# jagannatharjun/AntiZ

Hardware: AMD Instinct MI355X
Metric: input MB/s precompressed (1 GB synthetic, 100k streams) at 1/2/4/8 MI355X (higher is better)
Workload: dtype u8

## Files before the change

antiz_amd/__init__.py:

```python
import ctypes as C
import os

HERE = os.path.dirname(os.path.abspath(__file__))
LIB_PATH = os.environ.get("ATZ_LIB") or os.path.join(HERE, "_build", "libatz_accel.so")
CLI_PATH = os.path.join(HERE, "_build", "uncomp")

u64 = C.c_uint64
u8p = C.POINTER(C.c_uint8)


class Opts(C.Structure):
    _fields_ = [("recomp_tresh", u64), ("sizediff_tresh", u64), ("shortcut_len", u64), ("mismatch_tol", u64),
                ("chunksize", u64), ("brute_window", C.c_int32), ("device", C.c_int32)]


class Cand(C.Structure):
    _fields_ = [("offset", u64), ("comp_len", u64), ("infl_len", u64), ("type", C.c_int32), ("flags", C.c_uint32)]


class Result(C.Structure):
    _fields_ = [("clevel", C.c_uint8), ("window", C.c_uint8), ("memlevel", C.c_uint8), ("recomp", C.c_uint8),
                ("n_trials", C.c_uint32), ("ident", u64), ("first_diff", C.c_int64), ("n_diff", u64),
                ("diff_index", u64)]

# ... 12 lines not shown
                                   "trial_cyc_heap", "trial_cyc_fallback", "trial_symbols",
                                   "n_trials_speculative", "n_reinflated", "n_inflate_retries", "n_trials_replayed", "n_replay_checked",
                                   "n_trials_duplicate", "n_fast_restarts", "dev_bytes_peak", "dev_bytes_held",
                                   "n_trials_skipped")]

    def as_dict(self):
        return {k: getattr(self, k) for k, _ in self._fields_}


EXPORTS = ["atz_open", "atz_close", "atz_strerror", "atz_free", "atz_default_opts", "atz_scan", "atz_sweep",
           "atz_precompress", "atz_precompress_device", "atz_reconstruct", "atz_deflate", "atz_deflate_batch",
           "atz_inflate_batch", "atz_deflate_bound", "atz_shard_scan", "atz_shard_sweep", "atz_shard_piece",
           "atz_shard_assemble", "atz_reconstruct_device", "atz_deflate_batch_ex", "atz_set_strategies",
           "atz_set_containers", "atz_container_anchors", "atz_set_stitch", "atz_stitch_anchors",
           "atz_stitch_pieces", "atz_set_probe", "atz_probe_positions", "atz_set_deflaters",
           "atz_set_segments", "atz_flush_markers", "atz_inflate_segments"]

STRATEGIES = {"filtered": 1, "huffman": 2, "rle": 3}


def _mask(names, table, noun):
    if isinstance(names, str):
        names = [w for w in names.split(",") if w]
    mask = 0
    for w in names:
        if w not in table:
            raise ValueError("unknown %s %r (known: %s)" % (noun, w, ", ".join(sorted(table))))
        mask |= 1 << table[w]
    return mask


# ... 110 lines not shown
        L.atz_container_anchors.argtypes = [C.c_void_p, C.c_char_p, u64, C.c_uint32, C.POINTER(C.POINTER(u64)),
                                            C.POINTER(u64)]
        L.atz_set_stitch.argtypes = [C.c_void_p, C.c_uint32]
        L.atz_stitch_anchors.argtypes = L.atz_container_anchors.argtypes
        L.atz_stitch_pieces.argtypes = [C.c_void_p, u64, C.POINTER(C.POINTER(u64)), C.POINTER(C.POINTER(u64)),
                                        C.POINTER(u64)]
        L.atz_set_probe.argtypes = [C.c_void_p, C.c_uint32]
        L.atz_probe_positions.argtypes = [C.c_void_p, C.c_char_p, u64, C.POINTER(C.POINTER(u64)), C.POINTER(u64)]
        L.atz_set_deflaters.argtypes = [C.c_void_p, C.c_uint32]
        L.atz_set_segments.argtypes = [C.c_void_p, C.c_uint32]
        L.atz_flush_markers.argtypes = L.atz_probe_positions.argtypes
        L.atz_inflate_segments.argtypes = [C.c_void_p, C.c_char_p, u64, C.POINTER(u64), C.POINTER(u64), u64,
                                           C.POINTER(C.c_uint32), C.POINTER(u64), C.POINTER(u64), C.POINTER(C.c_uint8)]
        L.atz_deflate_bound.restype = u64
        L.atz_deflate_bound.argtypes = [u64, C.c_int, C.c_int]
        L.atz_shard_scan.argtypes = [C.c_void_p, C.c_void_p, C.c_char_p, u64, C.c_int, C.c_int, C.POINTER(u8p),
                                     C.POINTER(u64)]
        L.atz_shard_sweep.argtypes = [C.c_void_p, C.c_void_p, C.c_char_p, u64, C.POINTER(C.c_char_p),
                                      C.POINTER(u64), C.c_int, C.POINTER(u64), C.POINTER(u8p), C.POINTER(u64),
                                      C.POINTER(u64), C.POINTER(Stats)]
        L.atz_shard_piece.argtypes = [C.c_void_p, C.c_void_p]
        L.atz_reconstruct_device.argtypes = [C.c_void_p, C.c_void_p, C.c_char_p, u64, C.POINTER(C.c_void_p),
                                             C.POINTER(u64)]
        L.atz_shard_assemble.argtypes = [C.c_void_p, C.c_void_p, u64, C.c_char_p, u64, u64, u64, C.c_void_p, u64,
                                         C.POINTER(u64)]
        _lib = L
    return _lib


def _check(rc):
    if rc != 0:
        raise AtzError("atz error %d: %s" % (rc, lib().atz_strerror(rc).decode()), rc)


class Context:

    def __init__(self, recomp_tresh=128, sizediff_tresh=128, shortcut_len=512, mismatch_tol=2,
                 chunksize=524288, brute_window=False, device=-1, strategies=None, containers=None, stitch=None,
                 probe=None, deflaters=None, segments=None):
        L = lib()
        self.o = Opts(recomp_tresh, sizediff_tresh, shortcut_len, mismatch_tol, chunksize, int(brute_window), device)
        if strategies is None:
            strategies = os.environ.get("ATZ_STRATEGIES", "")
        mask = strategy_mask(strategies)
        if containers is None:
            containers = os.environ.get("ATZ_CONTAINERS", "")
        cmask = container_mask(containers)
# ... 235 lines not shown
```

antiz_amd/csrc/atz_accel.cpp:

```cpp
#include "k_inflate.hip"
#include "k_deflate.hip"

#include <algorithm>
#include <array>
#include <chrono>
#include <cstdio>
#include <cstdlib>
#include <cstring>
#include <deque>
#include <string>
#include <memory>
#include <new>
#include <stdexcept>
#include <atomic>
#include <thread>
#include <condition_variable>
#include <mutex>
#include <functional>
#include <unordered_map>
#include <vector>
#include <dlfcn.h>
#include <signal.h>
#include <sys/time.h>
#include <ucontext.h>
// ... 2105 lines not shown
      std::stable_sort(S.perm[k].begin(), S.perm[k].end(), [&](uint32_t a, uint32_t b) {
        const bool ma = mw_trial(c, k, in[k][a].memlevel), mb = mw_trial(c, k, in[k][b].memlevel);
        return ma != mb ? ma : key[a] > key[b];
      });
    }
    if (strat)
      std::stable_sort(S.perm[k].begin(), S.perm[k].end(), [&](uint32_t a, uint32_t b) {
        return trial_variant(c, k, in[k][a]) < trial_variant(c, k, in[k][b]);
      });
    S.tr[k].resize(n);
    for (size_t q = 0; q < n; q++) S.tr[k][q] = in[k][S.perm[k][q]];
    S.res[k].clear();
  }
  S.base = 0;
}
static int trials_launch(atz_ctx* x, Pipe* c, const uint8_t* d_cmp, const SweepOpts& so, int k, const Trial* h,
                         size_t cnt, size_t base) {
  struct Kern { int kind; uint32_t strat; bool mw; void (*fn)(SweepArgs); const char* name; };
  static const Kern kerns[] = {
      {0, 0, false, k_trial_stored, "k_trial_stored"},
      {0, 2, false, k_trial_huff, "k_trial_huff"},
      {0, 3, false, k_trial_rle, "k_trial_rle"},
      {1, 0, true, k_trial_fast_mw<BITMAP_BITS>, "k_trial_fast"},
      {1, 0, false, k_trial_fast<BITMAP_BITS>, "k_trial_fast"},
      {2, 0, true, k_trial_slow_mw, "k_trial_slow"},
      {2, 0, false, k_trial_slow, "k_trial_slow"},
      {2, 1, true, k_trial_slow_filt_mw, "k_trial_slow_filt"},
      {2, 1, false, k_trial_slow_filt, "k_trial_slow_filt"},
      {1, 4, false, k_trial_fast_gnu, "k_trial_fast_gnu"},
      {2, 4, false, k_trial_slow_gnu, "k_trial_slow_gnu"},
      {0, 8, false, k_trial_stored_flush, "k_trial_stored_flush"},
      {1, 8, true, k_trial_fast_flush_mw, "k_trial_fast_flush"},
      {1, 8, false, k_trial_fast_flush, "k_trial_fast_flush"},
      {2, 8, true, k_trial_slow_flush_mw, "k_trial_slow_flush"},
      {2, 8, false, k_trial_slow_flush, "k_trial_slow_flush"},
  };
  for (size_t i = 0; i < cnt; i++)
    if (h[i].host & (TH_WAITS | TH_DUP)) return ATZ_E_INTERNAL;
  for (size_t i = 0; i < cnt;) {
    const bool mw = mw_trial(c, k, h[i].memlevel);
    size_t j = i + 1;
    while (j < cnt && mw_trial(c, k, h[j].memlevel) == mw) j++;
    HIPCHK(pipe_copy(c, c->d_trials.as<Trial>() + base + i, h + i, (j - i) * sizeof(Trial), hipMemcpyHostToDevice));
    i = j;
  }
  auto launch1 = [&](const Trial* hh, size_t n1, size_t b1, uint32_t variant) -> int {
    (void)hh;
    const bool mw = variant & 1u;
    const Kern* kn = nullptr;
    for (const Kern& e : kerns)
      if (e.kind == k && e.strat == variant >> 1 && e.mw == mw) kn = &e;
    if (!kn) return ATZ_E_INTERNAL;
    SweepArgs A;
    A.file = d_cmp; A.infl = INFL_BASE; A.chains = CHAIN_BASE;
    A.R = c->d_R.as<uint2>();
    A.streams = x->d_streams.as<StreamDev>(); A.trials = c->d_trials.as<Trial>() + b1;
    A.res = c->d_tres.as<TrialRes>() + b1; A.out = c->d_out.as<uint8_t>(); A.syms = c->d_syms.as<uint32_t>();
    A.adler = x->d_adler.as<uint32_t>(); A.o = so; A.ntrials = (uint32_t)n1;
    A.stopj = c->stopj_cur;
    dim3 g((uint32_t)n1), b(mw ? MW_THREADS : 64);
    kbeg(c, variant & 8u ? 5 : 0);
    hipLaunchKernelGGL(kn->fn, g, b, 0, c->st, A);
    kend(c);
    KCHECK(kn->name);
    return 0;
// ... 2186 lines not shown
    uint64_t al = 0;
    auto tc = std::chrono::steady_clock::now();
    if (int r = precompress_dev(c, d_file, h_file, len, &al, nullptr)) return r;
    if (timing_on())
      std::fprintf(stderr, "atz: precompress call %.2f ms (inside: %.2f ms)\n", ms_since(tc), c->stats.total_ms);
    *d_atz = c->d_atz.as<uint8_t>();
    *atz_len = al;
    c->stats.dev_bytes_peak = g_dev.peak.load(); c->stats.dev_bytes_held = g_dev.cur.load();
    if (stats) *stats = c->stats;
    return ATZ_OK;
  });
}

uint64_t atz_deflate_bound(uint64_t n, int window, int memlevel) { return bound(n, window, memlevel); }

int atz_deflate(atz_ctx_t* c, const uint8_t* in, uint64_t in_len, int clevel, int window, int memlevel,
                uint8_t* out, uint64_t out_cap, uint64_t* out_len) {
  return guarded([&]() -> int {
    (void)hipGetLastError();
    if (!c || (!in && in_len) || !out_len || clevel < 0 || clevel > 9 || window < 8 || window > 15 ||
        memlevel < 1 || memlevel > 9)
      return ATZ_E_ARG;
    DeflSpec p;
    p.level = clevel; p.window = window == 8 ? 9 : window; p.memlevel = memlevel;
    std::vector<std::vector<uint8_t>> outs;
    if (int r = deflate_many(c, {{in, in_len}}, {p}, outs)) return r;
    *out_len = outs[0].size();
    if (outs[0].size() > out_cap) return ATZ_E_ARG;
    if (out && !outs[0].empty()) std::memcpy(out, outs[0].data(), outs[0].size());
    return ATZ_OK;
// ... 289 lines not shown
```

antiz_amd/csrc/k_deflate.hip:

```cpp
#include <hip/hip_runtime.h>
#include "atz_device.h"

#define LDS __attribute__((address_space(3)))
#define CONSTANT __attribute__((address_space(4)))
#define GLOBAL __attribute__((address_space(1)))

#ifndef ATZ_VISITED_CHECK
#define ATZ_VISITED_CHECK 1
#endif
#ifndef ATZ_VISITED_MAX
#define ATZ_VISITED_MAX 8
#endif
#ifndef ATZ_NOSLIDE_PATH
#define ATZ_NOSLIDE_PATH 1
#endif
#ifndef ATZ_STEP_SPLIT
#define ATZ_STEP_SPLIT 0
#endif
#ifndef ATZ_STEP_CLOCKS
#define ATZ_STEP_CLOCKS 0
#endif
#if ATZ_STEP_CLOCKS
#define STEP_CLOCK() clock64()
#else
// ... 696 lines not shown
      }
    }
    uint2 o;
    o.x = (bf > 2 ? (bf << 23) | (df << 8) : 0u) | s0;
    if (jb.fast) o.y = ((p - reach) << 16) | (budget_out << 12) | (slot << 1) | valid;
    else o.y = (bq > 2 ? (bq << 23) | (dq << 8) : 0u) | valid;
    r[p] = o;
  }
}

static constexpr int NLC = 286, NDC = 30, NBLC = 19, HEAPN = 2 * NLC + 1;
static constexpr uint32_t LOOKMIN = 262;
static constexpr uint32_t BITMAP_BITS = 32768;
static constexpr uint32_t HOLE_SLOTS = HOLE_SLOTS_M;

struct TreeWork {
  uint32_t heap[HEAPN + 1];
  uint16_t bl_count[16];
  uint32_t blc32[16];
};

struct TreeScratch {
  uint16_t anc[2][HEAPN];
  uint8_t dep[2][HEAPN];
  uint16_t freq[NLC];
};

struct BitOut {
  GLOBAL uint8_t* out;
  uint64_t cap;
  uint64_t pos;
  uint64_t bb;
  uint32_t bc;
  uint32_t raw;
  const GLOBAL uint8_t* orig;
  uint64_t clen;
  uint64_t shortcut;
  uint64_t eq_all;
  uint64_t eq_sc;
  int overflow;
  uint64_t cyc_tree, cyc_emit, blocks;
  uint64_t cyc_heap, cyc_scan, cyc_send;
};

static constexpr uint32_t STAGE_WORDS = 196;
struct BlockFreq {
  uint32_t lfreq2[(NLC + 1) / 2];
  uint32_t dfreq2[NDC / 2];
};
struct TreeCodes {
  uint16_t lcode[NLC]; uint8_t llen[NLC + 2];
  uint16_t dcode[NDC]; uint8_t dlen[NDC + 2];
  uint16_t bcode[NBLC]; uint8_t blen[NBLC + 2];
  uint32_t bfreq[NBLC];
  TreeWork w;
};
struct TrialShared {
  BitOut b;
  BlockFreq f;
  TreeCodes k;
  uint64_t stop_at;
  uint32_t stop_j, pad_;
};

template <uint32_t INS>
struct TrialSharedFast {
  static constexpr uint32_t INS_BITS = INS;
  TrialShared t;
  uint64_t ring[512];
  uint32_t ins[INS / 32];
  uint32_t holes[HOLE_SLOTS];
// ... 189 lines not shown
struct TreeRes {
  int max_code;
  uint64_t d_opt, d_static;
};

__device__ __noinline__ TreeRes build_tree(LDS TreeWork& w, LDS TreeScratch& sc, LDS uint8_t* lenv, int elems, int max_length, const CONSTANT uint8_t* xbits,
                                           int xbase, const CONSTANT uint8_t* stlen, LDS uint64_t& cyc_heap, int lane) {
  elems = (int)uni((uint32_t)elems);
  max_length = (int)uni((uint32_t)max_length);
  xbase = (int)uni((uint32_t)xbase);
  xbits = uni_ptr(xbits);
  stlen = uni_ptr(stlen);
  uint64_t opt_len = 0, static_len = 0;
  const uint64_t lt = lane ? (~0ull >> (64 - lane)) : 0ull;
  LDS uint32_t* const heap = w.heap;
  int heap_len = 0, max_code = -1;
  for (int g = 0; g < elems; g += 64) {
    const int n = g + lane;
    const uint32_t f = n < elems ? sc.freq[n] : 0u;
    const uint64_t m = __ballot(f != 0);
    if (f) heap[heap_len + 1 + __popcll(m & lt)] = tkey(f, 0, (uint32_t)n);
    else if (n < elems) lenv[n] = 0;
    if (m) max_code = g + 63 - __clzll((long long)m);
    heap_len += __popcll(m);
  }
  while (heap_len < 2) {
    const int node = max_code < 2 ? ++max_code : 0;
    ++heap_len;
    if (lane == 0) { heap[heap_len] = tkey(1, 0, (uint32_t)node); sc.freq[node] = 1; }
    opt_len--;
// ... 19 lines not shown
        go = vk > (hj >> 10);
        if (go) { wr(k, hj); k = j; j = k << 1; go = j <= len; }
      }
      wr(k, v);
    };
    for (int n = heap_len / 2; n >= 1; n--) down(heap_len, n);
    do {
      const uint32_t kn = rd(1);
      wr(1, rd(heap_len));
      wr(heap_len, 0xffffffffu);
      heap_len--;
      down(heap_len, 1);
      const uint32_t km = rd(1);
      const uint32_t dn = (kn >> 10) & 31u, dm = (km >> 10) & 31u;
      if (lane == 0) {
        heap[--heap_max] = kn & 1023u;
        heap[--heap_max] = km & 1023u;
        sc.anc[1][kn & 1023u] = (uint16_t)node;
        sc.anc[1][km & 1023u] = (uint16_t)node;
      } else {
        heap_max -= 2;
      }
      wr(1, tkey((kn >> 15) + (km >> 15), (dn >= dm ? dn : dm) + 1u, node));
      node++;
      down(heap_len, 1);
    } while (heap_len >= 2);
    root = rd(1) & 1023u;
  } else {
  for (int n = heap_len / 2; n >= 1; n--) pq_down(heap, heap_len, n, lane);
  do {
    const uint32_t kn = uni(heap[1]);
    heap[1] = uni(heap[heap_len]);
    heap_len--;
    pq_down(heap, heap_len, 1, lane);
    const uint32_t km = uni(heap[1]);
    const uint32_t dn = (kn >> 10) & 31u, dm = (km >> 10) & 31u;
    if (lane == 0) {
      heap[--heap_max] = kn & 1023u;
      heap[--heap_max] = km & 1023u;
      sc.anc[1][kn & 1023u] = (uint16_t)node;
      sc.anc[1][km & 1023u] = (uint16_t)node;
    } else {
      heap_max -= 2;
    }
    heap[1] = tkey((kn >> 15) + (km >> 15), (dn >= dm ? dn : dm) + 1u, node);
    node++;
    pq_down(heap, heap_len, 1, lane);
  } while (heap_len >= 2);
  root = uni(heap[1]) & 1023u;
  }
  if (lane == 0) cyc_heap += STEP_CLOCK() - ch0;
  --heap_max;
  if (lane == 0) heap[heap_max] = root;
  const int nn = (int)node;
  for (int i = lane; i < nn; i += 64) {
    const bool in_tree = i >= elems || (i <= max_code && sc.freq[i] != 0);
    const bool r = (uint32_t)i == root || !in_tree;
    sc.anc[0][i] = r ? (uint16_t)root : sc.anc[1][i];
    sc.dep[0][i] = r ? 0 : 1;
  }
  int cur = 0;
  for (int round = 0; round < 5; round++) {
    for (int i = lane; i < nn; i += 64) {
      const uint32_t a = sc.anc[cur][i];
      sc.dep[cur ^ 1][i] = (uint8_t)(sc.dep[cur][i] + sc.dep[cur][a]);
      sc.anc[cur ^ 1][i] = sc.anc[cur][a];
    }
    cur ^= 1;
  }
  if (lane < 16) w.blc32[lane] = 0;
  int overflow = 0;
  for (int g = 0; g < nn; g += 64) {
    const int i = g + lane;
    bool in_tree = false;
    uint32_t bits = 0;
    if (i < nn) {
      in_tree = i >= elems || (i <= max_code && sc.freq[i] != 0);
      bits = sc.dep[cur][i];
    }
    const bool capped = in_tree && (uint32_t)i != root && bits > (uint32_t)max_length;
    overflow += __popcll(__ballot(capped));
    if (bits > (uint32_t)max_length) bits = (uint32_t)max_length;
    const bool leaf = in_tree && i <= max_code;
    if (leaf) {
      lenv[i] = (uint8_t)bits;
      __hip_atomic_fetch_add(&w.blc32[bits], 1u, __ATOMIC_RELAXED, __HIP_MEMORY_SCOPE_WORKGROUP);
    }
  }
  uint32_t blc = lane >= 1 && lane < 16 ? w.blc32[lane] : 0u;
  if (overflow) {
    auto bl = [&](int b) -> uint32_t { return (uint32_t)__builtin_amdgcn_readlane((int)blc, b); };
    auto blset = [&](int b, uint32_t v) { blc = lane == b ? v : blc; };
    do {
      int bits = max_length - 1;
      while (bl(bits) == 0) bits--;
      blset(bits, bl(bits) - 1);
      blset(bits + 1, bl(bits + 1) + 2);
      blset(max_length, bl(max_length) - 1);
      overflow -= 2;
    } while (overflow > 0);
    int h = HEAPN;
    for (int bits = max_length; bits != 0; bits--) {
      uint32_t cnt = bl(bits);
      while (cnt != 0) {
        const uint32_t m = uni(heap[--h]);
        if ((int)m > max_code) continue;
        if (lane == 0) lenv[m] = (uint8_t)bits;
        cnt--;
      }
    }
  }
  if (lane < 16) w.bl_count[lane] = (uint16_t)blc;
  uint64_t o = 0, st = 0;
  for (int n = lane; n < elems && n <= max_code; n += 64) {
    const uint32_t f = sc.freq[n];
    if (f) {
      const uint32_t l = lenv[n];
      const uint32_t xb = (xbits && n >= xbase) ? xbits[n - xbase] : 0u;
      o += (uint64_t)f * (l + xb);
      if (stlen) st += (uint64_t)f * (stlen[n] + xb);
    }
  }
  opt_len += wsum64(o);
  if (stlen) static_len += wsum64(st);
  return TreeRes{max_code, opt_len, static_len};
}

__device__ __noinline__ void gen_codes(const LDS TreeWork& w, int max_code, LDS uint16_t* codes, LDS uint8_t* lens,
                                       int lane) {
  max_code = (int)uni((uint32_t)max_code);
  const bool lb = lane >= 1 && lane <= 15;
  const uint32_t bc = lb ? (uint32_t)w.bl_count[lane] : 0u;
  const uint32_t wv = bc << ((15 - lane) & 15);
  uint32_t nc = lb ? (wave_incl_scan(wv) - wv) >> (15 - lane) : 0u;
  const uint64_t lt = lane ? (~0ull >> (64 - lane)) : 0ull;
  const uint64_t present = __ballot(bc != 0);
  for (int g = 0; g <= max_code; g += 64) {
    const int n = g + lane;
    const uint32_t l = n <= max_code ? lens[n] : 0u;
    uint32_t mine = 0;
    for (uint64_t pm = present; pm; pm &= pm - 1) {
      const int b = __ffsll((unsigned long long)pm) - 1;
      const uint64_t m = __ballot(l == (uint32_t)b);
      if (!m) continue;
      const uint32_t base = (uint32_t)__builtin_amdgcn_readlane((int)nc, b);
      if (l == (uint32_t)b) mine = base + (uint32_t)__popcll(m & lt);
      if (lane == b) nc += (uint32_t)__popcll(m);
// ... 59 lines not shown
      if (xd) { v |= (uint64_t)(dist - dcode_base(dcd)) << nb; nb += xd; }
    }
  } else if (end) {
    v = lc[256]; nb = ll[256];
  }
}
__device__ __forceinline__ void stage_or(LDS uint32_t* stage, uint32_t off, uint64_t v, uint32_t nb) {
  if (!nb) return;
  const uint32_t wi = off >> 5, sh = off & 31;
  const uint64_t lo = v << sh;
  const uint32_t hi = sh ? (uint32_t)(v >> (64 - sh)) : 0;
  __atomic_fetch_or(&stage[wi], (uint32_t)lo, __ATOMIC_RELAXED);
  if ((uint32_t)(lo >> 32)) __atomic_fetch_or(&stage[wi + 1], (uint32_t)(lo >> 32), __ATOMIC_RELAXED);
  if (hi) __atomic_fetch_or(&stage[wi + 2], hi, __ATOMIC_RELAXED);
}
__device__ uint32_t rle_tree(LDS TreeCodes& s, LDS uint32_t* stage, const LDS uint8_t* ln, int max_code, bool send,
                             uint32_t off, int lane) {
  const int N = max_code + 1;
  const int G = N / 64 + 1;
  uint64_t M[5];
#pragma unroll
  for (int g = 0; g < 5; g++) {
    M[g] = 0;
    if (g < G) {
      const int n = 64 * g + lane;
      bool st = false;
      if (n == 0 || n == N) st = true;
      else if (n < N) st = ln[n] != ln[n - 1];
      M[g] = __ballot(st);
    }
  }
// ... 16 lines not shown
          const uint64_t m = h == g ? (M[h] & ~le) : M[h];
          if (m) en = 64 * h + __ffsll((unsigned long long)m) - 1;
        }
      const uint32_t v = ln[n];
      const int k = n - st, R = en - st;
      int cnt = 0, minc = 3;
      bool first = false;
      if (v != 0) {
        if (k == 0) { cnt = R < 7 ? R : 7; minc = 4; first = true; }
        else if (k >= 7 && (k - 7) % 6 == 0) cnt = R - k < 6 ? R - k : 6;
      } else if (k % 138 == 0) {
        cnt = R - k < 138 ? R - k : 138;
      }
      if (cnt) {
        if (!send) {
          if (cnt < minc) __atomic_fetch_add(&s.bfreq[v], (uint32_t)cnt, __ATOMIC_RELAXED);
          else if (v != 0) {
            if (first) __atomic_fetch_add(&s.bfreq[v], 1u, __ATOMIC_RELAXED);
            __atomic_fetch_add(&s.bfreq[16], 1u, __ATOMIC_RELAXED);
          } else __atomic_fetch_add(&s.bfreq[cnt <= 10 ? 17 : 18], 1u, __ATOMIC_RELAXED);
        } else {
          const uint32_t cv = s.bcode[v], cl = s.blen[v];
          if (cnt < minc) {
            for (int q = 0; q < cnt; q++) { v64 |= (uint64_t)cv << nb; nb += cl; }
          } else if (v != 0) {
            if (first) { v64 = cv; nb = cl; }
            v64 |= (uint64_t)s.bcode[16] << nb; nb += s.blen[16];
            v64 |= (uint64_t)(cnt - (first ? 1 : 0) - 3) << nb; nb += 2;
          } else if (cnt <= 10) {
            v64 = s.bcode[17]; nb = s.blen[17];
            v64 |= (uint64_t)(cnt - 3) << nb; nb += 3;
          } else {
            v64 = s.bcode[18]; nb = s.blen[18];
            v64 |= (uint64_t)(cnt - 11) << nb; nb += 7;
          }
        }
      }
    }
    if (send) {
      const uint32_t incl = wave_incl_scan(nb);
      stage_or(stage, off + incl - nb, v64, nb);
      off += (uint32_t)__builtin_amdgcn_readlane((int)incl, 63);
    }
  }
  return off;
}

template <typename C16, typename C8>
// ... 70 lines not shown
    }
  }
  return cap;
}

struct BlockPlan {
  uint64_t opt_lenb, static_lenb;
  int lmax, dmax, max_blindex;
};
__device__ __noinline__ BlockPlan block_trees(const LDS BlockFreq& f, LDS TreeCodes& s, LDS TreeScratch& sc, LDS uint64_t* cyc,
                                              uint32_t level, uint64_t stored_len, int lane) {
  level = uni(level);
  stored_len = uni(stored_len);
  BlockPlan pl{};
  uint64_t opt_len = 0, static_len = 0;
  if (level > 0) {
    for (int i = lane; i < NLC; i += 64) sc.freq[i] = (uint16_t)(f.lfreq2[i >> 1] >> (16 * (i & 1)));
    TreeRes r = build_tree(s.w, sc, s.llen, NLC, 15, (const CONSTANT uint8_t*)c_xlb, 257, (const CONSTANT uint8_t*)c_t.st_llen,
                           cyc[0], lane);
    pl.lmax = (int)uni((uint32_t)r.max_code);
    opt_len += uni(r.d_opt);
    static_len += uni(r.d_static);
    gen_codes(s.w, pl.lmax, s.lcode, s.llen, lane);
    for (int i = pl.lmax + 1 + lane; i < NLC + 2; i += 64) s.llen[i] = 0;
    for (int i = lane; i < NDC; i += 64) sc.freq[i] = (uint16_t)(f.dfreq2[i >> 1] >> (16 * (i & 1)));
    r = build_tree(s.w, sc, s.dlen, NDC, 15, (const CONSTANT uint8_t*)c_xdb, 0, (const CONSTANT uint8_t*)c_t.st_dlen,
                   cyc[0], lane);
    pl.dmax = (int)uni((uint32_t)r.max_code);
    opt_len += uni(r.d_opt);
    static_len += uni(r.d_static);
    gen_codes(s.w, pl.dmax, s.dcode, s.dlen, lane);
    for (int i = pl.dmax + 1 + lane; i < NDC + 2; i += 64) s.dlen[i] = 0;
    for (int i = lane; i < NBLC; i += 64) s.bfreq[i] = 0;
    const uint64_t cs0 = STEP_CLOCK();
    rle_tree(s, nullptr, s.llen, pl.lmax, false, 0, lane);
    rle_tree(s, nullptr, s.dlen, pl.dmax, false, 0, lane);
    if (lane == 0) cyc[1] += STEP_CLOCK() - cs0;
    for (int i = lane; i < NBLC; i += 64) sc.freq[i] = (uint16_t)s.bfreq[i];
    r = build_tree(s.w, sc, s.blen, NBLC, 7, (const CONSTANT uint8_t*)c_xblb, 0, nullptr, cyc[0], lane);
    const int bmax = (int)uni((uint32_t)r.max_code);
    opt_len += uni(r.d_opt);
    gen_codes(s.w, bmax, s.bcode, s.blen, lane);
    for (int i = bmax + 1 + lane; i < NBLC + 2; i += 64) s.blen[i] = 0;
    int mb;
    for (mb = NBLC - 1; mb >= 3; mb--)
      if (s.blen[bl_order((uint32_t)mb)] != 0) break;
    pl.max_blindex = mb;
    opt_len += 3 * ((uint64_t)mb + 1) + 5 + 5 + 4;
    pl.opt_lenb = (opt_len + 3 + 7) >> 3;
    pl.static_lenb = (static_len + 3 + 7) >> 3;
    if (pl.static_lenb <= pl.opt_lenb) pl.opt_lenb = pl.static_lenb;
  } else {
    pl.opt_lenb = pl.static_lenb = stored_len + 5;
  }
  return pl;
}

// ... 42 lines not shown
        }
        stage[k] = wv;
      }
      emit_bytes_from_stage(b, stage, nb, lane);
      if (!full_needed && early_exit(b, opt, best_ident, false) != ~0u) break;
    }
  } else if (static_lenb == opt_lenb) {
    const uint32_t bc0 = uni(b.bc);
    b.bb = uni(b.bb) | ((uint64_t)((1u << 1) + (uint32_t)last) << bc0);
    b.bc = bc0 + 3;
    compress_block(b, stage, syms, last_lit, (const CONSTANT uint16_t*)c_t.st_lcode, (const CONSTANT uint8_t*)c_t.st_llen,
                   (const CONSTANT uint16_t*)c_t.st_dcode, (const CONSTANT uint8_t*)c_t.st_dlen, opt, best_ident,
                   full_needed, lane);
  } else {
    int lcodes = lmax + 1, dcodes = dmax + 1, blcodes = max_blindex + 1;
    const uint64_t cs0 = STEP_CLOCK();
    for (int i = lane; i < (int)STAGE_WORDS; i += 64) stage[i] = 0;
    const uint32_t bc0 = uni(b.bc);
    const uint64_t bb0 = uni(b.bb);
    if (lane == 0) { stage[0] = (uint32_t)bb0; stage[1] = (uint32_t)(bb0 >> 32); }
    uint32_t off = bc0;
    if (lane == 0)
      stage_or(stage, off, (uint64_t)((2u << 1) + (uint32_t)last) | ((uint64_t)(lcodes - 257) << 3) |
                               ((uint64_t)(dcodes - 1) << 8) | ((uint64_t)(blcodes - 4) << 13), 17);
    off += 17;
    if (lane < blcodes) stage_or(stage, off + 3u * (uint32_t)lane, s.blen[bl_order((uint32_t)lane)], 3);
    off += 3u * (uint32_t)blcodes;
    off = rle_tree(s, stage, s.llen, lcodes - 1, true, off, lane);
    off = rle_tree(s, stage, s.dlen, dcodes - 1, true, off, lane);
    {
      const uint32_t full = off >> 3;
      emit_bytes_from_stage(b, stage, full, lane);
      const uint32_t rem = off & 7;
      const uint32_t lastw = stage[full >> 2];
      b.bb = rem ? ((lastw >> (8 * (full & 3))) & 0xff) & ((1u << rem) - 1) : 0;
      b.bc = rem;
    }
    b.cyc_send += STEP_CLOCK() - cs0;
    compress_block(b, stage, syms, last_lit, (const LDS uint16_t*)s.lcode, (const LDS uint8_t*)s.llen,
                   (const LDS uint16_t*)s.dcode, (const LDS uint8_t*)s.dlen, opt, best_ident, full_needed, lane);
  }
  if (b.pos - blk_start_bytes > (uint64_t)lbs + 2ull * last_lit && last_lit) hazard = 1;
  if (last) windup(b, stage, lane);
  return hazard;
}

__device__ __forceinline__ void init_block(LDS BlockFreq& f, int lane) {
  for (int i = lane; i < (NLC + 1) / 2; i += 64) f.lfreq2[i] = 0;
  for (int i = lane; i < NDC / 2; i += 64) f.dfreq2[i] = 0;
  if (lane == 0) f.lfreq2[128] = 1;
}

__device__ __forceinline__ uint32_t flush_block(LDS TrialShared& s, LDS TreeScratch& sc, LDS BitOut& b, const GLOBAL uint32_t* syms,
                                                const GLOBAL uint8_t* in, int64_t block_start, uint64_t p, uint64_t S,
                                                uint32_t last_lit, uint32_t level, uint32_t lbs, int last, const SweepOpts& opt,
// ... 1212 lines not shown
      if (lane == 0) {
        TrialRes r = {};
        r.state = TR_SKIPPED;
        A.res[blockIdx.x] = r;
      }
      return;
    }
  }
  TrialRun<KIND, SH, STRAT, FAM> run(A, shm, lane);
  run.run();
}

#ifndef TRIAL_SLOW_WAVES
#define TRIAL_SLOW_WAVES 4
#endif
__global__ __launch_bounds__(64, TRIAL_SLOW_WAVES) void k_trial_stored(SweepArgs A) {
  __shared__ struct { TrialShared t; uint64_t ring[(STAGE_WORDS + 1) / 2]; } shm;
  trial_body<0>(A, shm, threadIdx.x);
}
template <uint32_t INS>
__global__ __launch_bounds__(64, TRIAL_SLOW_WAVES) void k_trial_fast(SweepArgs A) {
  __shared__ TrialSharedFast<INS> shm;
  trial_body<1>(A, shm, threadIdx.x);
}
__global__ __launch_bounds__(64, TRIAL_SLOW_WAVES) void k_trial_slow(SweepArgs A) {
  __shared__ TrialSharedSlow shm;
  trial_body<2>(A, shm, threadIdx.x);
}
static constexpr uint32_t MW_THREADS = 64 * (1 + MW_F);
template <uint32_t INS>
__global__ __launch_bounds__(MW_THREADS, TRIAL_SLOW_WAVES) void k_trial_fast_mw(SweepArgs A) {
  __shared__ TrialSharedFastMW<INS> shm;
  trial_body<1>(A, shm, (int)(threadIdx.x & 63));
}
__global__ __launch_bounds__(MW_THREADS, TRIAL_SLOW_WAVES) void k_trial_slow_mw(SweepArgs A) {
  __shared__ TrialSharedSlowMW shm;
  trial_body<2>(A, shm, (int)(threadIdx.x & 63));
}
__global__ __launch_bounds__(64, TRIAL_SLOW_WAVES) void k_trial_slow_filt(SweepArgs A) {
  __shared__ TrialSharedSlow shm;
  trial_body<2, TrialSharedSlow, 1>(A, shm, threadIdx.x);
}
__global__ __launch_bounds__(MW_THREADS, TRIAL_SLOW_WAVES) void k_trial_slow_filt_mw(SweepArgs A) {
  __shared__ TrialSharedSlowMW shm;
  trial_body<2, TrialSharedSlowMW, 1>(A, shm, (int)(threadIdx.x & 63));
}
__global__ __launch_bounds__(64, TRIAL_SLOW_WAVES) void k_trial_rle(SweepArgs A) {
  __shared__ TrialSharedSlow shm;
  trial_body<3>(A, shm, threadIdx.x);
}
__global__ __launch_bounds__(64, TRIAL_SLOW_WAVES) void k_trial_huff(SweepArgs A) {
  __shared__ TrialSharedSlow shm;
  trial_body<4>(A, shm, threadIdx.x);
}
__global__ __launch_bounds__(64, TRIAL_SLOW_WAVES) void k_trial_fast_gnu(SweepArgs A) {
  __shared__ TrialSharedFast<BITMAP_BITS> shm;
  trial_body<1, TrialSharedFast<BITMAP_BITS>, 0, 1>(A, shm, threadIdx.x);
}
__global__ __launch_bounds__(64, TRIAL_SLOW_WAVES) void k_trial_slow_gnu(SweepArgs A) {
  __shared__ TrialSharedSlow shm;
  trial_body<2, TrialSharedSlow, 0, 1>(A, shm, threadIdx.x);
}
__global__ __launch_bounds__(64, TRIAL_SLOW_WAVES) void k_trial_stored_flush(SweepArgs A) {
  __shared__ struct { TrialShared t; uint64_t ring[(STAGE_WORDS + 1) / 2]; } shm;
  trial_body<0, decltype(shm), 0, 2>(A, shm, threadIdx.x);
}
__global__ __launch_bounds__(64, TRIAL_SLOW_WAVES) void k_trial_fast_flush(SweepArgs A) {
  __shared__ TrialSharedFast<BITMAP_BITS> shm;
  trial_body<1, TrialSharedFast<BITMAP_BITS>, 0, 2>(A, shm, threadIdx.x);
}
__global__ __launch_bounds__(64, TRIAL_SLOW_WAVES) void k_trial_slow_flush(SweepArgs A) {
  __shared__ TrialSharedSlow shm;
  trial_body<2, TrialSharedSlow, 0, 2>(A, shm, threadIdx.x);
}
__global__ __launch_bounds__(MW_THREADS, TRIAL_SLOW_WAVES) void k_trial_fast_flush_mw(SweepArgs A) {
  __shared__ TrialSharedFastMW<BITMAP_BITS> shm;
  trial_body<1, TrialSharedFastMW<BITMAP_BITS>, 0, 2>(A, shm, (int)(threadIdx.x & 63));
}
__global__ __launch_bounds__(MW_THREADS, TRIAL_SLOW_WAVES) void k_trial_slow_flush_mw(SweepArgs A) {
  __shared__ TrialSharedSlowMW shm;
  trial_body<2, TrialSharedSlowMW, 0, 2>(A, shm, (int)(threadIdx.x & 63));
}

}
```

include/atz_accel.h:

```cpp
#ifndef ATZ_ACCEL_H
#define ATZ_ACCEL_H
#include <stdint.h>
#ifdef __cplusplus
extern "C" {
#endif

typedef struct atz_ctx atz_ctx_t;

typedef struct {
    uint64_t recomp_tresh;
    uint64_t sizediff_tresh;
    uint64_t shortcut_len;
    uint64_t mismatch_tol;
    uint64_t chunksize;
    int32_t  brute_window;
    int32_t  device;
} atz_opts_t;

typedef struct {
    uint64_t offset;
    uint64_t comp_len;
    uint64_t infl_len;
    int32_t  type;
    uint32_t flags;
// ... 109 lines not shown
int atz_inflate_batch(atz_ctx_t *ctx, const uint8_t *buf, uint64_t len, const uint64_t *offs,
                      const uint64_t *lens, uint64_t n, uint32_t *status, uint64_t *consumed, uint64_t *produced);

int atz_shard_scan(atz_ctx_t *ctx, const uint8_t *d_file, const uint8_t *h_file, uint64_t len, int rank, int world,
                   uint8_t **blob, uint64_t *blob_len);
int atz_shard_sweep(atz_ctx_t *ctx, const uint8_t *d_file, const uint8_t *h_file, uint64_t len,
                    const uint8_t *const *blobs, const uint64_t *blob_lens, int world, uint64_t *piece_len,
                    uint8_t **recomp_flags, uint64_t *n_flags, uint64_t *n_recomp, atz_stats_t *stats);
int atz_shard_piece(atz_ctx_t *ctx, uint8_t *d_dst);
int atz_shard_assemble(atz_ctx_t *ctx, const uint8_t *d_file, uint64_t len, const uint8_t *recomp_flags,
                       uint64_t n_flags, uint64_t n_recomp, uint64_t pieces_len, uint8_t *d_atz, uint64_t cap,
                       uint64_t *atz_len);

uint64_t atz_deflate_bound(uint64_t n, int window, int memlevel);

#ifdef __cplusplus
}
#endif
#endif
```

Before: 1669.

## Shrink tree LDS footprint and raise lazy trial kernels' occupancy bound

Huffman tree work space shrinks. The heap node list is stored as 16-bit entries packed above the key words. The code words are moved into an unused region of the tree scratch's ancestor array, and the separate 16-bit bl_count is merged with the 32-bit one. The LDS saved lets the slow, filtered, rle, huff and flush trial kernels declare a higher minimum-waves launch bound (5 instead of 4), aiming for more resident blocks per CU. A query for trial-kernel occupancy is added for inspection. The aliasing of code words into scratch depends on careful lifetime reasoning, and the tighter launch bound may force register spills.

```diff
diff --git a/antiz_amd/__init__.py b/antiz_amd/__init__.py
--- a/antiz_amd/__init__.py
+++ b/antiz_amd/__init__.py
@@ -50,7 +50,7 @@
            "atz_shard_assemble", "atz_reconstruct_device", "atz_deflate_batch_ex", "atz_set_strategies",
            "atz_set_containers", "atz_container_anchors", "atz_set_stitch", "atz_stitch_anchors",
            "atz_stitch_pieces", "atz_set_probe", "atz_probe_positions", "atz_set_deflaters",
-           "atz_set_segments", "atz_flush_markers", "atz_inflate_segments"]
+           "atz_set_segments", "atz_flush_markers", "atz_inflate_segments", "atz_trial_occupancy"]
 
 STRATEGIES = {"filtered": 1, "huffman": 2, "rle": 3}
 
@@ -191,6 +191,8 @@
                                            C.POINTER(C.c_uint32), C.POINTER(u64), C.POINTER(u64), C.POINTER(C.c_uint8)]
         L.atz_deflate_bound.restype = u64
         L.atz_deflate_bound.argtypes = [u64, C.c_int, C.c_int]
+        if hasattr(L, "atz_trial_occupancy"):
+            L.atz_trial_occupancy.argtypes = [C.c_char_p, C.POINTER(C.c_int)]
         L.atz_shard_scan.argtypes = [C.c_void_p, C.c_void_p, C.c_char_p, u64, C.c_int, C.c_int, C.POINTER(u8p),
                                      C.POINTER(u64)]
         L.atz_shard_sweep.argtypes = [C.c_void_p, C.c_void_p, C.c_char_p, u64, C.POINTER(C.c_char_p),
@@ -208,6 +210,12 @@
 def _check(rc):
     if rc != 0:
         raise AtzError("atz error %d: %s" % (rc, lib().atz_strerror(rc).decode()), rc)
+
+
+def trial_occupancy(kernel):
+    n = C.c_int(0)
+    _check(lib().atz_trial_occupancy(kernel.encode(), C.byref(n)))
+    return n.value
 
 
 class Context:
diff --git a/antiz_amd/csrc/atz_accel.cpp b/antiz_amd/csrc/atz_accel.cpp
--- a/antiz_amd/csrc/atz_accel.cpp
+++ b/antiz_amd/csrc/atz_accel.cpp
@@ -2143,27 +2143,27 @@
   }
   S.base = 0;
 }
+struct TrialKern { int kind; uint32_t strat; bool mw; void (*fn)(SweepArgs); const char* name; };
+static const TrialKern trial_kerns[] = {
+    {0, 0, false, k_trial_stored, "k_trial_stored"},
+    {0, 2, false, k_trial_huff, "k_trial_huff"},
+    {0, 3, false, k_trial_rle, "k_trial_rle"},
+    {1, 0, true, k_trial_fast_mw<BITMAP_BITS>, "k_trial_fast"},
+    {1, 0, false, k_trial_fast<BITMAP_BITS>, "k_trial_fast"},
+    {2, 0, true, k_trial_slow_mw, "k_trial_slow"},
+    {2, 0, false, k_trial_slow, "k_trial_slow"},
+    {2, 1, true, k_trial_slow_filt_mw, "k_trial_slow_filt"},
+    {2, 1, false, k_trial_slow_filt, "k_trial_slow_filt"},
+    {1, 4, false, k_trial_fast_gnu, "k_trial_fast_gnu"},
+    {2, 4, false, k_trial_slow_gnu, "k_trial_slow_gnu"},
+    {0, 8, false, k_trial_stored_flush, "k_trial_stored_flush"},
+    {1, 8, true, k_trial_fast_flush_mw, "k_trial_fast_flush"},
+    {1, 8, false, k_trial_fast_flush, "k_trial_fast_flush"},
+    {2, 8, true, k_trial_slow_flush_mw, "k_trial_slow_flush"},
+    {2, 8, false, k_trial_slow_flush, "k_trial_slow_flush"},
+};
 static int trials_launch(atz_ctx* x, Pipe* c, const uint8_t* d_cmp, const SweepOpts& so, int k, const Trial* h,
                          size_t cnt, size_t base) {
-  struct Kern { int kind; uint32_t strat; bool mw; void (*fn)(SweepArgs); const char* name; };
-  static const Kern kerns[] = {
-      {0, 0, false, k_trial_stored, "k_trial_stored"},
-      {0, 2, false, k_trial_huff, "k_trial_huff"},
-      {0, 3, false, k_trial_rle, "k_trial_rle"},
-      {1, 0, true, k_trial_fast_mw<BITMAP_BITS>, "k_trial_fast"},
-      {1, 0, false, k_trial_fast<BITMAP_BITS>, "k_trial_fast"},
-      {2, 0, true, k_trial_slow_mw, "k_trial_slow"},
-      {2, 0, false, k_trial_slow, "k_trial_slow"},
-      {2, 1, true, k_trial_slow_filt_mw, "k_trial_slow_filt"},
-      {2, 1, false, k_trial_slow_filt, "k_trial_slow_filt"},
-      {1, 4, false, k_trial_fast_gnu, "k_trial_fast_gnu"},
-      {2, 4, false, k_trial_slow_gnu, "k_trial_slow_gnu"},
-      {0, 8, false, k_trial_stored_flush, "k_trial_stored_flush"},
-      {1, 8, true, k_trial_fast_flush_mw, "k_trial_fast_flush"},
-      {1, 8, false, k_trial_fast_flush, "k_trial_fast_flush"},
-      {2, 8, true, k_trial_slow_flush_mw, "k_trial_slow_flush"},
-      {2, 8, false, k_trial_slow_flush, "k_trial_slow_flush"},
-  };
   for (size_t i = 0; i < cnt; i++)
     if (h[i].host & (TH_WAITS | TH_DUP)) return ATZ_E_INTERNAL;
   for (size_t i = 0; i < cnt;) {
@@ -2176,8 +2176,8 @@
   auto launch1 = [&](const Trial* hh, size_t n1, size_t b1, uint32_t variant) -> int {
     (void)hh;
     const bool mw = variant & 1u;
-    const Kern* kn = nullptr;
-    for (const Kern& e : kerns)
+    const TrialKern* kn = nullptr;
+    for (const TrialKern& e : trial_kerns)
       if (e.kind == k && e.strat == variant >> 1 && e.mw == mw) kn = &e;
     if (!kn) return ATZ_E_INTERNAL;
     SweepArgs A;
@@ -4394,6 +4394,22 @@
 
 uint64_t atz_deflate_bound(uint64_t n, int window, int memlevel) { return bound(n, window, memlevel); }
 
+int atz_trial_occupancy(const char* kernel, int* blocks_per_cu) {
+  return guarded([&]() -> int {
+    (void)hipGetLastError();
+    if (!kernel || !blocks_per_cu) return ATZ_E_ARG;
+    std::string name(kernel);
+    const bool mw = name.size() > 3 && name.compare(name.size() - 3, 3, "_mw") == 0;
+    if (mw) name.resize(name.size() - 3);
+    for (const TrialKern& e : trial_kerns)
+      if (e.mw == mw && name == e.name) {
+        HIPCHK(hipOccupancyMaxActiveBlocksPerMultiprocessor(blocks_per_cu, (const void*)e.fn, mw ? (int)MW_THREADS : 64, 0));
+        return ATZ_OK;
+      }
+    return ATZ_E_ARG;
+  });
+}
+
 int atz_deflate(atz_ctx_t* c, const uint8_t* in, uint64_t in_len, int clevel, int window, int memlevel,
                 uint8_t* out, uint64_t out_cap, uint64_t* out_len) {
   return guarded([&]() -> int {
diff --git a/antiz_amd/csrc/k_deflate.hip b/antiz_amd/csrc/k_deflate.hip
--- a/antiz_amd/csrc/k_deflate.hip
+++ b/antiz_amd/csrc/k_deflate.hip
@@ -734,11 +734,13 @@
 static constexpr uint32_t BITMAP_BITS = 32768;
 static constexpr uint32_t HOLE_SLOTS = HOLE_SLOTS_M;
 
+static constexpr int HEAP_WORDS = NLC + 2;
+static_assert(2 * HEAP_WORDS >= HEAPN && NLC < HEAP_WORDS, "the key words stay below the node list");
 struct TreeWork {
-  uint32_t heap[HEAPN + 1];
-  uint16_t bl_count[16];
-  uint32_t blc32[16];
+  uint32_t heap[HEAP_WORDS];
+  uint32_t bl_count[16];
 };
+__device__ __forceinline__ LDS uint16_t* heap_nodes(LDS TreeWork& w) { return (LDS uint16_t*)w.heap + (2 * HEAP_WORDS - HEAPN); }
 
 struct TreeScratch {
   uint16_t anc[2][HEAPN];
@@ -769,12 +771,24 @@
   uint32_t dfreq2[NDC / 2];
 };
 struct TreeCodes {
-  uint16_t lcode[NLC]; uint8_t llen[NLC + 2];
-  uint16_t dcode[NDC]; uint8_t dlen[NDC + 2];
-  uint16_t bcode[NBLC]; uint8_t blen[NBLC + 2];
-  uint32_t bfreq[NBLC];
+  uint8_t llen[NLC + 2];
+  uint8_t dlen[NDC + 2];
+  uint8_t blen[NBLC + 2];
   TreeWork w;
 };
+struct TreeCodeWords {
+  uint16_t lcode[NLC], dcode[NDC], bcode[NBLC];
+  uint32_t bfreq[NBLC];
+};
+static constexpr uint32_t CODES_OFF = 1272;
+static_assert(CODES_OFF % alignof(TreeCodeWords) == 0, "TreeCodeWords' place in the tree scratch");
+static_assert(CODES_OFF >= STAGE_WORDS * 4, "the codes are read while the staging words are written");
+static_assert(CODES_OFF >= offsetof(TreeScratch, anc) + sizeof(uint16_t) * (HEAPN + 2 * NDC) && 2 * NBLC <= 2 * NDC,
+              "the distance and bit-length trees' nodes stay below the codes");
+static_assert(CODES_OFF + sizeof(TreeCodeWords) <= offsetof(TreeScratch, dep), "the codes lie within anc[1]");
+__device__ __forceinline__ LDS TreeCodeWords& code_words(LDS TreeScratch& sc) {
+  return *(LDS TreeCodeWords*)((LDS uint8_t*)&sc + CODES_OFF);
+}
 struct TrialShared {
   BitOut b;
   BlockFreq f;
@@ -994,6 +1008,7 @@
   uint64_t opt_len = 0, static_len = 0;
   const uint64_t lt = lane ? (~0ull >> (64 - lane)) : 0ull;
   LDS uint32_t* const heap = w.heap;
+  LDS uint16_t* const nodes = heap_nodes(w);
   int heap_len = 0, max_code = -1;
   for (int g = 0; g < elems; g += 64) {
     const int n = g + lane;
@@ -1043,8 +1058,8 @@
       const uint32_t km = rd(1);
       const uint32_t dn = (kn >> 10) & 31u, dm = (km >> 10) & 31u;
       if (lane == 0) {
-        heap[--heap_max] = kn & 1023u;
-        heap[--heap_max] = km & 1023u;
+        nodes[--heap_max] = (uint16_t)(kn & 1023u);
+        nodes[--heap_max] = (uint16_t)(km & 1023u);
         sc.anc[1][kn & 1023u] = (uint16_t)node;
         sc.anc[1][km & 1023u] = (uint16_t)node;
       } else {
@@ -1065,8 +1080,8 @@
     const uint32_t km = uni(heap[1]);
     const uint32_t dn = (kn >> 10) & 31u, dm = (km >> 10) & 31u;
     if (lane == 0) {
-      heap[--heap_max] = kn & 1023u;
-      heap[--heap_max] = km & 1023u;
+      nodes[--heap_max] = (uint16_t)(kn & 1023u);
+      nodes[--heap_max] = (uint16_t)(km & 1023u);
       sc.anc[1][kn & 1023u] = (uint16_t)node;
       sc.anc[1][km & 1023u] = (uint16_t)node;
     } else {
@@ -1080,7 +1095,7 @@
   }
   if (lane == 0) cyc_heap += STEP_CLOCK() - ch0;
   --heap_max;
-  if (lane == 0) heap[heap_max] = root;
+  if (lane == 0) nodes[heap_max] = (uint16_t)root;
   const int nn = (int)node;
   for (int i = lane; i < nn; i += 64) {
     const bool in_tree = i >= elems || (i <= max_code && sc.freq[i] != 0);
@@ -1097,7 +1112,7 @@
     }
     cur ^= 1;
   }
-  if (lane < 16) w.blc32[lane] = 0;
+  if (lane < 16) w.bl_count[lane] = 0;
   int overflow = 0;
   for (int g = 0; g < nn; g += 64) {
     const int i = g + lane;
@@ -1113,10 +1128,10 @@
     const bool leaf = in_tree && i <= max_code;
     if (leaf) {
       lenv[i] = (uint8_t)bits;
-      __hip_atomic_fetch_add(&w.blc32[bits], 1u, __ATOMIC_RELAXED, __HIP_MEMORY_SCOPE_WORKGROUP);
-    }
-  }
-  uint32_t blc = lane >= 1 && lane < 16 ? w.blc32[lane] : 0u;
+      __hip_atomic_fetch_add(&w.bl_count[bits], 1u, __ATOMIC_RELAXED, __HIP_MEMORY_SCOPE_WORKGROUP);
+    }
+  }
+  uint32_t blc = lane >= 1 && lane < 16 ? w.bl_count[lane] : 0u;
   if (overflow) {
     auto bl = [&](int b) -> uint32_t { return (uint32_t)__builtin_amdgcn_readlane((int)blc, b); };
     auto blset = [&](int b, uint32_t v) { blc = lane == b ? v : blc; };
@@ -1132,14 +1147,14 @@
     for (int bits = max_length; bits != 0; bits--) {
       uint32_t cnt = bl(bits);
       while (cnt != 0) {
-        const uint32_t m = uni(heap[--h]);
+        const uint32_t m = uni((uint32_t)nodes[--h]);
         if ((int)m > max_code) continue;
         if (lane == 0) lenv[m] = (uint8_t)bits;
         cnt--;
       }
     }
   }
-  if (lane < 16) w.bl_count[lane] = (uint16_t)blc;
+  if (lane < 16) w.bl_count[lane] = blc;
   uint64_t o = 0, st = 0;
   for (int n = lane; n < elems && n <= max_code; n += 64) {
     const uint32_t f = sc.freq[n];
@@ -1159,7 +1174,7 @@
                                        int lane) {
   max_code = (int)uni((uint32_t)max_code);
   const bool lb = lane >= 1 && lane <= 15;
-  const uint32_t bc = lb ? (uint32_t)w.bl_count[lane] : 0u;
+  const uint32_t bc = lb ? w.bl_count[lane] : 0u;
   const uint32_t wv = bc << ((15 - lane) & 15);
   uint32_t nc = lb ? (wave_incl_scan(wv) - wv) >> (15 - lane) : 0u;
   const uint64_t lt = lane ? (~0ull >> (64 - lane)) : 0ull;
@@ -1249,7 +1264,7 @@
   if ((uint32_t)(lo >> 32)) __atomic_fetch_or(&stage[wi + 1], (uint32_t)(lo >> 32), __ATOMIC_RELAXED);
   if (hi) __atomic_fetch_or(&stage[wi + 2], hi, __ATOMIC_RELAXED);
 }
-__device__ uint32_t rle_tree(LDS TreeCodes& s, LDS uint32_t* stage, const LDS uint8_t* ln, int max_code, bool send,
+__device__ uint32_t rle_tree(LDS TreeCodes& s, LDS TreeCodeWords& cw, LDS uint32_t* stage, const LDS uint8_t* ln, int max_code, bool send,
                              uint32_t off, int lane) {
   const int N = max_code + 1;
   const int G = N / 64 + 1;
@@ -1296,24 +1311,24 @@
       }
       if (cnt) {
         if (!send) {
-          if (cnt < minc) __atomic_fetch_add(&s.bfreq[v], (uint32_t)cnt, __ATOMIC_RELAXED);
+          if (cnt < minc) __atomic_fetch_add(&cw.bfreq[v], (uint32_t)cnt, __ATOMIC_RELAXED);
           else if (v != 0) {
-            if (first) __atomic_fetch_add(&s.bfreq[v], 1u, __ATOMIC_RELAXED);
-            __atomic_fetch_add(&s.bfreq[16], 1u, __ATOMIC_RELAXED);
-          } else __atomic_fetch_add(&s.bfreq[cnt <= 10 ? 17 : 18], 1u, __ATOMIC_RELAXED);
+            if (first) __atomic_fetch_add(&cw.bfreq[v], 1u, __ATOMIC_RELAXED);
+            __atomic_fetch_add(&cw.bfreq[16], 1u, __ATOMIC_RELAXED);
+          } else __atomic_fetch_add(&cw.bfreq[cnt <= 10 ? 17 : 18], 1u, __ATOMIC_RELAXED);
         } else {
-          const uint32_t cv = s.bcode[v], cl = s.blen[v];
+          const uint32_t cv = cw.bcode[v], cl = s.blen[v];
           if (cnt < minc) {
             for (int q = 0; q < cnt; q++) { v64 |= (uint64_t)cv << nb; nb += cl; }
           } else if (v != 0) {
             if (first) { v64 = cv; nb = cl; }
-            v64 |= (uint64_t)s.bcode[16] << nb; nb += s.blen[16];
+            v64 |= (uint64_t)cw.bcode[16] << nb; nb += s.blen[16];
             v64 |= (uint64_t)(cnt - (first ? 1 : 0) - 3) << nb; nb += 2;
           } else if (cnt <= 10) {
-            v64 = s.bcode[17]; nb = s.blen[17];
+            v64 = cw.bcode[17]; nb = s.blen[17];
             v64 |= (uint64_t)(cnt - 3) << nb; nb += 3;
           } else {
-            v64 = s.bcode[18]; nb = s.blen[18];
+            v64 = cw.bcode[18]; nb = s.blen[18];
             v64 |= (uint64_t)(cnt - 11) << nb; nb += 7;
           }
         }
@@ -1414,6 +1429,7 @@
   stored_len = uni(stored_len);
   BlockPlan pl{};
   uint64_t opt_len = 0, static_len = 0;
+  LDS TreeCodeWords& cw = code_words(sc);
   if (level > 0) {
     for (int i = lane; i < NLC; i += 64) sc.freq[i] = (uint16_t)(f.lfreq2[i >> 1] >> (16 * (i & 1)));
     TreeRes r = build_tree(s.w, sc, s.llen, NLC, 15, (const CONSTANT uint8_t*)c_xlb, 257, (const CONSTANT uint8_t*)c_t.st_llen,
@@ -1421,7 +1437,7 @@
     pl.lmax = (int)uni((uint32_t)r.max_code);
     opt_len += uni(r.d_opt);
     static_len += uni(r.d_static);
-    gen_codes(s.w, pl.lmax, s.lcode, s.llen, lane);
+    gen_codes(s.w, pl.lmax, cw.lcode, s.llen, lane);
     for (int i = pl.lmax + 1 + lane; i < NLC + 2; i += 64) s.llen[i] = 0;
     for (int i = lane; i < NDC; i += 64) sc.freq[i] = (uint16_t)(f.dfreq2[i >> 1] >> (16 * (i & 1)));
     r = build_tree(s.w, sc, s.dlen, NDC, 15, (const CONSTANT uint8_t*)c_xdb, 0, (const CONSTANT uint8_t*)c_t.st_dlen,
@@ -1429,18 +1445,18 @@
     pl.dmax = (int)uni((uint32_t)r.max_code);
     opt_len += uni(r.d_opt);
     static_len += uni(r.d_static);
-    gen_codes(s.w, pl.dmax, s.dcode, s.dlen, lane);
+    gen_codes(s.w, pl.dmax, cw.dcode, s.dlen, lane);
     for (int i = pl.dmax + 1 + lane; i < NDC + 2; i += 64) s.dlen[i] = 0;
-    for (int i = lane; i < NBLC; i += 64) s.bfreq[i] = 0;
+    for (int i = lane; i < NBLC; i += 64) cw.bfreq[i] = 0;
     const uint64_t cs0 = STEP_CLOCK();
-    rle_tree(s, nullptr, s.llen, pl.lmax, false, 0, lane);
-    rle_tree(s, nullptr, s.dlen, pl.dmax, false, 0, lane);
+    rle_tree(s, cw, nullptr, s.llen, pl.lmax, false, 0, lane);
+    rle_tree(s, cw, nullptr, s.dlen, pl.dmax, false, 0, lane);
     if (lane == 0) cyc[1] += STEP_CLOCK() - cs0;
-    for (int i = lane; i < NBLC; i += 64) sc.freq[i] = (uint16_t)s.bfreq[i];
+    for (int i = lane; i < NBLC; i += 64) sc.freq[i] = (uint16_t)cw.bfreq[i];
     r = build_tree(s.w, sc, s.blen, NBLC, 7, (const CONSTANT uint8_t*)c_xblb, 0, nullptr, cyc[0], lane);
     const int bmax = (int)uni((uint32_t)r.max_code);
     opt_len += uni(r.d_opt);
-    gen_codes(s.w, bmax, s.bcode, s.blen, lane);
+    gen_codes(s.w, bmax, cw.bcode, s.blen, lane);
     for (int i = bmax + 1 + lane; i < NBLC + 2; i += 64) s.blen[i] = 0;
     int mb;
     for (mb = NBLC - 1; mb >= 3; mb--)
@@ -1513,6 +1529,7 @@
                    full_needed, lane);
   } else {
     int lcodes = lmax + 1, dcodes = dmax + 1, blcodes = max_blindex + 1;
+    LDS TreeCodeWords& cw = code_words(*(LDS TreeScratch*)stage);
     const uint64_t cs0 = STEP_CLOCK();
     for (int i = lane; i < (int)STAGE_WORDS; i += 64) stage[i] = 0;
     const uint32_t bc0 = uni(b.bc);
@@ -1525,8 +1542,8 @@
     off += 17;
     if (lane < blcodes) stage_or(stage, off + 3u * (uint32_t)lane, s.blen[bl_order((uint32_t)lane)], 3);
     off += 3u * (uint32_t)blcodes;
-    off = rle_tree(s, stage, s.llen, lcodes - 1, true, off, lane);
-    off = rle_tree(s, stage, s.dlen, dcodes - 1, true, off, lane);
+    off = rle_tree(s, cw, stage, s.llen, lcodes - 1, true, off, lane);
+    off = rle_tree(s, cw, stage, s.dlen, dcodes - 1, true, off, lane);
     {
       const uint32_t full = off >> 3;
       emit_bytes_from_stage(b, stage, full, lane);
@@ -1536,8 +1553,8 @@
       b.bc = rem;
     }
     b.cyc_send += STEP_CLOCK() - cs0;
-    compress_block(b, stage, syms, last_lit, (const LDS uint16_t*)s.lcode, (const LDS uint8_t*)s.llen,
-                   (const LDS uint16_t*)s.dcode, (const LDS uint8_t*)s.dlen, opt, best_ident, full_needed, lane);
+    compress_block(b, stage, syms, last_lit, (const LDS uint16_t*)cw.lcode, (const LDS uint8_t*)s.llen,
+                   (const LDS uint16_t*)cw.dcode, (const LDS uint8_t*)s.dlen, opt, best_ident, full_needed, lane);
   }
   if (b.pos - blk_start_bytes > (uint64_t)lbs + 2ull * last_lit && last_lit) hazard = 1;
   if (last) windup(b, stage, lane);
@@ -2780,6 +2797,9 @@
 #ifndef TRIAL_SLOW_WAVES
 #define TRIAL_SLOW_WAVES 4
 #endif
+#ifndef TRIAL_LAZY_WAVES
+#define TRIAL_LAZY_WAVES 5
+#endif
 __global__ __launch_bounds__(64, TRIAL_SLOW_WAVES) void k_trial_stored(SweepArgs A) {
   __shared__ struct { TrialShared t; uint64_t ring[(STAGE_WORDS + 1) / 2]; } shm;
   trial_body<0>(A, shm, threadIdx.x);
@@ -2789,7 +2809,7 @@
   __shared__ TrialSharedFast<INS> shm;
   trial_body<1>(A, shm, threadIdx.x);
 }
-__global__ __launch_bounds__(64, TRIAL_SLOW_WAVES) void k_trial_slow(SweepArgs A) {
+__global__ __launch_bounds__(64, TRIAL_LAZY_WAVES) void k_trial_slow(SweepArgs A) {
   __shared__ TrialSharedSlow shm;
   trial_body<2>(A, shm, threadIdx.x);
 }
@@ -2799,23 +2819,23 @@
   __shared__ TrialSharedFastMW<INS> shm;
   trial_body<1>(A, shm, (int)(threadIdx.x & 63));
 }
-__global__ __launch_bounds__(MW_THREADS, TRIAL_SLOW_WAVES) void k_trial_slow_mw(SweepArgs A) {
+__global__ __launch_bounds__(MW_THREADS, TRIAL_LAZY_WAVES) void k_trial_slow_mw(SweepArgs A) {
   __shared__ TrialSharedSlowMW shm;
   trial_body<2>(A, shm, (int)(threadIdx.x & 63));
 }
-__global__ __launch_bounds__(64, TRIAL_SLOW_WAVES) void k_trial_slow_filt(SweepArgs A) {
+__global__ __launch_bounds__(64, TRIAL_LAZY_WAVES) void k_trial_slow_filt(SweepArgs A) {
   __shared__ TrialSharedSlow shm;
   trial_body<2, TrialSharedSlow, 1>(A, shm, threadIdx.x);
 }
-__global__ __launch_bounds__(MW_THREADS, TRIAL_SLOW_WAVES) void k_trial_slow_filt_mw(SweepArgs A) {
+__global__ __launch_bounds__(MW_THREADS, TRIAL_LAZY_WAVES) void k_trial_slow_filt_mw(SweepArgs A) {
   __shared__ TrialSharedSlowMW shm;
   trial_body<2, TrialSharedSlowMW, 1>(A, shm, (int)(threadIdx.x & 63));
 }
-__global__ __launch_bounds__(64, TRIAL_SLOW_WAVES) void k_trial_rle(SweepArgs A) {
+__global__ __launch_bounds__(64, TRIAL_LAZY_WAVES) void k_trial_rle(SweepArgs A) {
   __shared__ TrialSharedSlow shm;
   trial_body<3>(A, shm, threadIdx.x);
 }
-__global__ __launch_bounds__(64, TRIAL_SLOW_WAVES) void k_trial_huff(SweepArgs A) {
+__global__ __launch_bounds__(64, TRIAL_LAZY_WAVES) void k_trial_huff(SweepArgs A) {
   __shared__ TrialSharedSlow shm;
   trial_body<4>(A, shm, threadIdx.x);
 }
@@ -2835,7 +2855,7 @@
   __shared__ TrialSharedFast<BITMAP_BITS> shm;
   trial_body<1, TrialSharedFast<BITMAP_BITS>, 0, 2>(A, shm, threadIdx.x);
 }
-__global__ __launch_bounds__(64, TRIAL_SLOW_WAVES) void k_trial_slow_flush(SweepArgs A) {
+__global__ __launch_bounds__(64, TRIAL_LAZY_WAVES) void k_trial_slow_flush(SweepArgs A) {
   __shared__ TrialSharedSlow shm;
   trial_body<2, TrialSharedSlow, 0, 2>(A, shm, threadIdx.x);
 }
@@ -2843,7 +2863,7 @@
   __shared__ TrialSharedFastMW<BITMAP_BITS> shm;
   trial_body<1, TrialSharedFastMW<BITMAP_BITS>, 0, 2>(A, shm, (int)(threadIdx.x & 63));
 }
-__global__ __launch_bounds__(MW_THREADS, TRIAL_SLOW_WAVES) void k_trial_slow_flush_mw(SweepArgs A) {
+__global__ __launch_bounds__(MW_THREADS, TRIAL_LAZY_WAVES) void k_trial_slow_flush_mw(SweepArgs A) {
   __shared__ TrialSharedSlowMW shm;
   trial_body<2, TrialSharedSlowMW, 0, 2>(A, shm, (int)(threadIdx.x & 63));
 }
diff --git a/include/atz_accel.h b/include/atz_accel.h
--- a/include/atz_accel.h
+++ b/include/atz_accel.h
@@ -147,6 +147,8 @@
 
 uint64_t atz_deflate_bound(uint64_t n, int window, int memlevel);
 
+int atz_trial_occupancy(const char *kernel, int *blocks_per_cu);
+
 #ifdef __cplusplus
 }
 #endif
```

Result: no change. 1686, median of 2 (+1.1%).
